# apple/ml-stable-diffusion

Measured on AMD Instinct MI355X. Metric: diffusion iter/s (UNet steps/s), SD2.1-base 512x512 fp16, higher is better.
Workload: dtype fp16; 1 GPU; BASELINE config 2: SD2.1-base (865.9 M-parameter UNet), random-init, denoising iteration at 512x512 (64x64 latents), CFG batch 2 per prompt, DDIM, device-resident loop; unet=sd21-base, latent=64, attention=ORIGINAL, prompts_per_gpu=1, global_batch=2, hip_graph=True, parallelism=dp1 (independent prompts per rank, no data-path collective)

## Files before the change

ml-stable-diffusion_amd/csrc/capi.cpp:

```cpp
#include <cmath>
#include <cstdlib>
#include <cstring>

#include "unet.h"

namespace sd {
extern thread_local std::string g_last_error;
int selftest_mfma();

namespace {

template <typename F>
int guarded(F&& f) {
  try {
    f();
    g_last_error.clear();
    return kOk;
  } catch (const Error& e) {
    g_last_error = e.what();
    return e.code;
  } catch (const std::bad_alloc&) {
    g_last_error = "out of host memory";
    return kInternal;
  } catch (const std::exception& e) {
    g_last_error = e.what();
    return kInternal;
  }
}

void require_device() {
  int n = 0;
  hipError_t e = hipGetDeviceCount(&n);
  if (e != hipSuccess || n <= 0)
    fail(kHipError, "no HIP device visible (%s): libsdmi355 has no CPU fallback", hipGetErrorString(e));
}

struct Scratch {
  std::vector<void*> ptrs;
  hipStream_t stream = nullptr;
  hipEvent_t e0 = nullptr, e1 = nullptr;
  Scratch() {
    require_device();
    SD_HIP(hipStreamCreateWithFlags(&stream, hipStreamNonBlocking));
    SD_HIP(hipEventCreate(&e0));
    SD_HIP(hipEventCreate(&e1));
  }
  ~Scratch() {
    if (stream) (void)hipStreamSynchronize(stream);
    for (void* p : ptrs) (void)hipFree(p);
    if (e0) (void)hipEventDestroy(e0);
    if (e1) (void)hipEventDestroy(e1);
    if (stream) (void)hipStreamDestroy(stream);
  }
  template <typename T>
  T* dev(size_t n, const T* host = nullptr) {
    void* p = nullptr;
    SD_HIP(hipMalloc(&p, std::max<size_t>(n, 1) * sizeof(T)));
    ptrs.push_back(p);
    if (host)
      SD_HIP(hipMemcpy(p, host, n * sizeof(T), hipMemcpyHostToDevice));
    else
      SD_HIP(hipMemset(p, 0, std::max<size_t>(n, 1) * sizeof(T)));
    return reinterpret_cast<T*>(p);
  }
  template <typename F>
  void timed(int iters, float* ms, F&& launch) {
    if (iters < 1) iters = 1;
    static const bool poison = tune_env_set("SD_POISON_LDS");
    if (poison) {
      launch();
      launch_lds_poison(stream);
      launch();
      SD_HIP(hipStreamSynchronize(stream));
      if (ms) *ms = 0.f;
      return;
    }
    launch();
    SD_HIP(hipStreamSynchronize(stream));
    static const bool cold = tune_env_set("SD_BENCH_COLD");
    if (cold) {
      const size_t flush_bytes = (size_t)512 << 20;
      void* flush = dev<char>(flush_bytes);
// ... 936 lines not shown
      auto gemm_res = [&](const half_t* in, int cin, const half_t* w, const float* bias, const half_t* res, half_t* dst) {
        ConvDesc cd;
        cd.x0 = in; cd.C0 = cin; cd.w = w; cd.bias = bias; cd.res = res; cd.out = dst;
        cd.B = B; cd.Hi = 1; cd.Wi = S; cd.Ho = 1; cd.Wo = S; cd.N = C;
        SD_REQUIRE(conv_fast_path_ok(cd), kInvalidArgument, "ffn_out_proj: off the MFMA path");
        return cd;
      };
      ConvDesc c1 = gemm_res(dg, K1, dw1, db1, dr1, dh3);
      ConvDesc c2 = gemm_res(dh3, C, dw2, db2, dr2, o);
      c2.gn_partial = partial;
      c2.gn_groups = groups;
      ConvWorkspace ws;
      ws.partial_bytes = std::max(conv_workspace_bytes(c1), conv_workspace_bytes(c2));
      if (ws.partial_bytes) ws.partial = reinterpret_cast<float*>(sc.dev<char>(ws.partial_bytes));
      sc.timed(iters, ms, [&] {
        launch_conv(c1, ws, sc.stream);
        n_entries = launch_conv(c2, ws, sc.stream);
      });
    }
    std::vector<half_t> ot((size_t)M * C);
    SD_HIP(hipMemcpy(ot.data(), o, ot.size() * 2, hipMemcpyDeviceToHost));
    half_t* oh = reinterpret_cast<half_t*>(out);
    for (int b = 0; b < B; ++b)
      for (int c = 0; c < C; ++c)
        for (int s = 0; s < S; ++s) oh[((size_t)b * C + c) * S + s] = ot[((size_t)b * S + s) * C + c];
    if (gn_sums) {
      std::vector<float> hp(pf);
      SD_HIP(hipMemcpy(hp.data(), partial, pf * sizeof(float), hipMemcpyDeviceToHost));
      for (int b = 0; b < B; ++b)
        for (int gi = 0; gi < groups; ++gi) {
          double s1 = 0.0, s2 = 0.0;
          for (int e = 0; e < n_entries; ++e) {
            s1 += hp[(((size_t)b * groups + gi) * kGnMaxSlabs + e) * 2];
            s2 += hp[(((size_t)b * groups + gi) * kGnMaxSlabs + e) * 2 + 1];
          }
          gn_sums[((size_t)b * groups + gi) * 2] = n_entries ? (float)s1 : NAN;
          gn_sums[((size_t)b * groups + gi) * 2 + 1] = n_entries ? (float)s2 : NAN;
        }
    }
  });
}

int sd_op_geglu(const void* x, const void* w, const float* bias, void* out, int M, int C, int N2, int iters, float* ms) {
  return guarded([&] {
    SD_REQUIRE(x && w && out && N2 % 2 == 0, kInvalidArgument, "bad GEGLU arguments");
    Scratch sc;
    const half_t* wh = reinterpret_cast<const half_t*>(w);
    const int half_n = N2 / 2;
    SD_REQUIRE(half_n % 32 == 0, kUnsupported, "GEGLU needs (N/2) %% 32 == 0");
    std::vector<half_t> wt((size_t)N2 * C);
    std::vector<float> bt(N2, 0.f);
    for (int o = 0; o < N2; ++o) {
      const bool gate = o >= half_n;
      const int j = gate ? o - half_n : o;
      const int dst = (j / 32) * 64 + (gate ? 32 : 0) + (j % 32);
      std::memcpy(&wt[(size_t)dst * C], &wh[(size_t)o * C], (size_t)C * 2);
      if (bias) bt[dst] = bias[o];
    }
    ConvDesc d;
    d.x0 = sc.dev<half_t>((size_t)M * C, reinterpret_cast<const half_t*>(x));
    d.C0 = C;
    d.w = sc.dev<half_t>(wt.size(), wt.data());
    d.bias = bias ? sc.dev<float>(N2, bt.data()) : nullptr;
    half_t* dout = sc.dev<half_t>((size_t)M * half_n);
    d.out = dout;
    d.B = 1; d.Hi = 1; d.Wi = M; d.Ho = 1; d.Wo = M;
    d.N = N2;
    d.out_mode = kOutGeglu;
    const bool fast = conv_fast_path_ok(d);
    ConvWorkspace ws;
    sc.timed(iters, ms, [&] {
      if (fast)
        launch_conv(d, ws, sc.stream);
      else
        launch_conv_generic(d, 0, sc.stream);
    });
    SD_HIP(hipMemcpy(out, dout, (size_t)M * half_n * 2, hipMemcpyDeviceToHost));
  });
}

int sd_op_geglu_ln(const void* x, const float* ln_weight, const float* ln_bias, const void* w, const float* bias, void* out, int M, int C,
                   int N2, float eps, int kernel, int iters, float* ms) {
  return guarded([&] {
    const int abl = kernel / 10;
    kernel %= 10;
    SD_REQUIRE(x && w && out && N2 % 64 == 0 && (ln_weight == nullptr) == (ln_bias == nullptr) && kernel >= 0 && kernel <= 9 &&
                   (abl == 0 || kernel == 2), kInvalidArgument, "bad GEGLU arguments");
    Scratch sc;
    const half_t* wh = reinterpret_cast<const half_t*>(w);
    const int half_n = N2 / 2;
    std::vector<half_t> wt((size_t)N2 * C);
    std::vector<float> bt(N2, 0.f), cst(N2, 0.f);
    for (int o = 0; o < N2; ++o) {
      const bool gate = o >= half_n;
      const int j = gate ? o - half_n : o;
      const int dst = (j / 32) * 64 + (gate ? 32 : 0) + (j % 32);
      double cs = 0.0, bb = bias ? (double)bias[o] : 0.0;
      for (int c = 0; c < C; ++c) {
        const float wv = (float)wh[(size_t)o * C + c];
        const half_t h = ln_weight ? (half_t)(wv * ln_weight[c]) : wh[(size_t)o * C + c];
        wt[(size_t)dst * C + c] = h;
        cs += (double)(float)h;
        if (ln_bias) bb += (double)wv * (double)ln_bias[c];
      }
      bt[dst] = (float)bb;
      cst[dst] = (float)cs;
    }
    ConvDesc d;
    d.x0 = sc.dev<half_t>((size_t)M * C, reinterpret_cast<const half_t*>(x));
    d.C0 = C;
    d.w = sc.dev<half_t>(wt.size(), wt.data());
    d.bias = sc.dev<float>(N2, bt.data());
    if (ln_weight) d.ln_colsum = sc.dev<float>(N2, cst.data());
    d.ln_eps = eps;
    half_t* dout = sc.dev<half_t>((size_t)M * half_n);
    d.out = dout;
    d.B = 1; d.Hi = 1; d.Wi = M; d.Ho = 1; d.Wo = M;
    d.N = N2;
    d.out_mode = kOutGeglu;
    SD_REQUIRE(conv_fast_path_ok(d), kUnsupported, "GEGLU shape off the MFMA path (C=%d N2=%d)", C, N2);
    if (kernel != 1 && kernel < 3 && wsgemm_shape_ok(d)) {
      half_t* wtd = sc.dev<half_t>(wsgemm_tiled_halves(N2));
      launch_wsgemm_retile(d.w, wtd, N2, true, sc.stream);
      d.w_ws = wtd;
    }
    if (kernel == 2) d.tile = 10;
    if (kernel >= 3) {
      SD_REQUIRE(bvgemm_shape_ok(d), kInvalidArgument, "GEGLU shape not eligible for plan tile 11 (bvgemm.hip)");
      half_t* wtd = sc.dev<half_t>(bvgemm_tiled_halves(N2, C));
      launch_bvgemm_retile(d.w, wtd, N2, C, true, sc.stream);
      d.w_bv = wtd;
      d.w_ws = nullptr;
      d.tile = 11;
      d.staging = kernel - 3;
    }
    d.debug = abl;
    if (abl == 5) d.prof = sc.dev<long long>(64);
    ConvWorkspace ws;
    sc.timed(iters, ms, [&] { launch_conv(d, ws, sc.stream); });
    if (d.prof) {
      long long t[64];
      SD_HIP(hipMemcpy(t, d.prof, sizeof(t), hipMemcpyDeviceToHost));
      for (int i = 0; i < 6; ++i)
        fprintf(stderr, "[sd prof] wsgemm iteration %d: barrier wait %lld, DMA issue + store %lld, statistics %lld, MFMA || epilogue %lld cycles\n",
                i + 1, t[i * 8 + 1] - t[i * 8], t[i * 8 + 2] - t[i * 8 + 1], t[i * 8 + 3] - t[i * 8 + 2], t[i * 8 + 4] - t[i * 8 + 3]);
    }
    SD_HIP(hipMemcpy(out, dout, (size_t)M * half_n * 2, hipMemcpyDeviceToHost));
  });
}

int sd_op_qkv_ln(const void* x, const float* ln_weight, const float* ln_bias, const void* w, void* out_qk, void* out_vt, int B, int HW, int C,
                 float eps, float q_scale, int vt_perm, int kernel, int iters, float* ms) {
  return guarded([&] {
    SD_REQUIRE(x && ln_weight && ln_bias && w && out_qk && out_vt && B >= 1 && HW >= 1 && C % 64 == 0 && kernel >= 0 && kernel <= 9,
               kInvalidArgument, "bad q|k|v arguments");
    Scratch sc;
    const half_t* wh = reinterpret_cast<const half_t*>(w);
    const int N = 3 * C, M = B * HW;
    std::vector<half_t> wt((size_t)N * C);
    std::vector<float> bt(N, 0.f), cst(N, 0.f);
    for (int o = 0; o < N; ++o) {
      double cs = 0.0, bb = 0.0;
      for (int c = 0; c < C; ++c) {
        const float wv = (float)wh[(size_t)o * C + c];
        const half_t h = (half_t)(wv * ln_weight[c]);
        wt[(size_t)o * C + c] = h;
        cs += (double)(float)h;
        bb += (double)wv * (double)ln_bias[c];
      }
      bt[o] = (float)bb;
      cst[o] = (float)cs;
    }
    ConvDesc d;
    d.x0 = sc.dev<half_t>((size_t)M * C, reinterpret_cast<const half_t*>(x));
    d.C0 = C;
    d.w = sc.dev<half_t>(wt.size(), wt.data());
    d.bias = sc.dev<float>(N, bt.data());
    d.ln_colsum = sc.dev<float>(N, cst.data());
    d.ln_eps = eps;
    half_t* dqk = sc.dev<half_t>((size_t)M * 2 * C);
    half_t* dvt = sc.dev<half_t>((size_t)B * C * HW);
    d.out = dqk;
    d.out_t = dvt;
    d.n_trans = 2 * C;
    d.ldT = HW;
    d.vt_perm = vt_perm ? 1 : 0;
    d.q_scale = q_scale;
    d.q_cols = C;
    d.B = B; d.Hi = 1; d.Wi = HW; d.Ho = 1; d.Wo = HW;
    d.N = N;
    SD_REQUIRE(conv_fast_path_ok(d), kUnsupported, "q|k|v shape off the MFMA path (C=%d)", C);
    if (kernel == 2 || (kernel == 0 && wsgemm_wanted(d))) {
      SD_REQUIRE(wsgemm_shape_ok(d), kInvalidArgument, "q|k|v shape not eligible for plan tile 10 (wsgemm.hip)");
      half_t* wtd = sc.dev<half_t>(wsgemm_tiled_halves(N));
      launch_wsgemm_retile(d.w, wtd, N, false, sc.stream);
      d.w_ws = wtd;
      if (kernel == 2) d.tile = 10;
    } else if (kernel >= 3 || (kernel == 0 && bvgemm_wanted(d))) {
      SD_REQUIRE(bvgemm_shape_ok(d), kInvalidArgument, "q|k|v shape not eligible for plan tile 11 (bvgemm.hip)");
      half_t* wtd = sc.dev<half_t>(bvgemm_tiled_halves(N, C));
      launch_bvgemm_retile(d.w, wtd, N, C, false, sc.stream);
      d.w_bv = wtd;
      if (kernel >= 3) {
        d.tile = 11;
        d.staging = kernel - 3;
      }
    }
    ConvWorkspace ws;
    sc.timed(iters, ms, [&] { launch_conv(d, ws, sc.stream); });
    SD_HIP(hipMemcpy(out_qk, dqk, (size_t)M * 2 * C * 2, hipMemcpyDeviceToHost));
    SD_HIP(hipMemcpy(out_vt, dvt, (size_t)B * C * HW * 2, hipMemcpyDeviceToHost));
  });
}

int sd_op_gn_proj_qkv(const void* x_in, const void* conv_w, const float* gn_weight, const float* gn_bias, const void* proj_w,
                      const float* proj_bias, const float* ln_weight, const float* ln_bias, const void* wqkv, void* out_h, void* out_qk,
                      void* out_vt, int B, int H, int W, int C, int groups, float gn_eps, float ln_eps, float q_scale, int vt_perm, int fused,
                      int* entries, int iters, float* ms) {
  return guarded([&] {
    SD_REQUIRE(x_in && conv_w && gn_weight && gn_bias && proj_w && proj_bias && ln_weight && ln_bias && wqkv && out_h && out_qk && out_vt,
               kInvalidArgument, "NULL argument");
    const int HW = H * W, M = B * HW, N = 3 * C;
    SD_REQUIRE(gn_proj_qkv_ok(C, C / 64, HW, M, HW, groups), kInvalidArgument, "gn_proj_qkv: C=%d HW=%d groups=%d", C, HW, groups);
// ... 276 lines not shown
```

ml-stable-diffusion_amd/csrc/igemm.hip:

```cpp
#include <cstdio>
#include <cstdlib>
#include <cstring>
#include <string>
#include <type_traits>

#include "kernels.h"

namespace sd {

namespace {

constexpr int BK = 64;
constexpr int LDS_ROW = BK + 8;

struct IgemmArgs {
  const half_t* x0;
  const half_t* x1;
  const half_t* w;
  const float* bias;
  const float* temb;
  const half_t* res;
  half_t* out;
  float* partial;
  int C0, C1, Ctot;
// ... 2407 lines not shown
    int ppb = std::max(1, a.B * a.HoWo / 512);
    const int slabs = cdiv(a.HoWo, ppb);
    const size_t lds = (size_t)ppb * (a.N / 4) * 2 * sizeof(float);
    if (slabs <= kGnMaxSlabs && lds <= 64 * 1024) {
      a.gn_partial = d.gn_partial;
      a.gn_G = d.gn_groups;
      a.gn_cpg = a.N / d.gn_groups;
      a.gn_T = slabs;
      hipLaunchKernelGGL(splitk_reduce_stats_kernel, dim3(slabs, a.B), dim3(256), lds, s, a, ppb);
      return slabs;
    }
  }
  const size_t total4 = (size_t)a.M * a.N / 4;
  const int blocks = (int)std::min<size_t>((total4 + 255) / 256, 2048);
  hipLaunchKernelGGL(splitk_reduce_kernel, dim3(blocks), dim3(256), 0, s, a);
  return 0;
}
}

namespace {
void choose_tile_order(IgemmArgs& a, int tile) {
  int bm, bn;
  tile_dims(tile, bm, bn);
  const bool halo_tile = tile == 7;
  const double nbn = (double)cdiv(a.N, bn);
  const double nbm = halo_tile ? (double)a.B * a.tiles_x * a.tiles_y : (double)cdiv(a.M, bm);
  const double a_bytes = 2.0 * a.B * a.Hi * a.Wi * a.Ctot, w_bytes = 2.0 * a.N * a.K;
  const double l2 = 3.5e6;
  const double m_fast_cost = w_bytes + a_bytes * (a_bytes <= l2 ? std::min(8.0, nbn) : nbn);
  const double n_fast_cost = a_bytes + w_bytes * (w_bytes <= l2 ? std::min(8.0, nbm) : nbm);
  static const int forced = tune_env_int("SD_TILE_ORDER", -1);
  if (forced == 2) a.n_fast = nbn > 1 && a_bytes * (nbn - 1) > 7.0 * w_bytes;
  else a.n_fast = forced >= 0 ? (forced != 0) : (nbn > 1 && n_fast_cost < m_fast_cost);
}
}

bool conv_gn_loader_ok(const ConvDesc& d) {
  const int c1 = d.x1 ? d.C1 : 0;
  const int ctot = d.C0 + c1;
  return d.ksize == 3 && d.stride == 1 && d.up == 1 && halo_ks_ok(d) && !d.ln_colsum && !d.out_t && d.out_mode == kOutHalf && !d.debug &&
         d.gnf_groups >= 1 && d.gnf_groups <= 32 && ctot % d.gnf_groups == 0 && ctot <= 2048 && d.Hi == d.Ho && d.Wi == d.Wo &&
         halo_gnl_lds_bytes(3, ctot) <= halo_gnl_lds_cap;
}

int launch_conv(const ConvDesc& d, const ConvWorkspace& ws, hipStream_t s) {
  SD_REQUIRE(conv_fast_path_ok(d), kInvalidArgument, "launch_conv: shape not MFMA-tileable (C0=%d C1=%d N=%d k=%d)",
             d.C0, d.C1, d.N, d.ksize);
  SD_REQUIRE(!d.ln_colsum || (d.ksize == 1 && !d.x1 && d.bias && d.out_mode != kOutHalfT), kInvalidArgument,
             "LayerNorm fold needs a 1x1 single-source GEMM with a (folded) bias");
  SD_REQUIRE(!d.out_t || (d.out_mode == kOutHalf && d.n_trans % 64 == 0 && d.n_trans < d.N && (d.Ho * d.Wo) % 8 == 0 &&
                          d.ldT % 8 == 0 && !d.res && !d.temb),
             kInvalidArgument, "fused q|k|v: n_trans %d N %d HoWo %d ldT %d", d.n_trans, d.N, d.Ho * d.Wo, d.ldT);
  SD_REQUIRE(!d.vt_perm || (d.out_t && (d.Ho * d.Wo) % 16 == 0), kInvalidArgument, "permuted V^T needs the fused q|k|v epilogue and HoWo %% 16 == 0");
  SD_REQUIRE(d.q_cols == 0 || (d.out_t && d.q_cols % 4 == 0 && d.q_cols <= d.n_trans), kInvalidArgument, "pre-scaled queries need the fused q|k|v epilogue (q_cols %d)", d.q_cols);
  {
    static const bool wsg_on = tune_env_int("SD_WSGEMM", 1) != 0;
    const bool forced = d.tile == 10;
    if (d.w_ws && wsgemm_shape_ok(d) && (forced || (wsg_on && wsgemm_wanted(d) && d.tile == 0 && d.splitk == 0 && d.staging == 0 && g_tune.tile == 0))) {
      launch_wsgemm(d, s);
      return 0;
    }
    SD_REQUIRE(!forced, kInvalidArgument, "plan tile 10 (wsgemm.hip) needs the pre-tiled weights and an eligible GEGLU shape");
  }
  {
    static const bool bv_on = tune_env_int("SD_BVGEMM", 1) != 0;
    if (bv_on && d.w_bv && d.tile == 0 && d.splitk == 0 && d.staging == 0 && g_tune.tile == 0 && bvgemm_wanted(d)) {
      launch_bvgemm(d, 0, s);
      return 0;
    }
  }
  if (d.tile == 11) {
    SD_REQUIRE(d.w_bv && bvgemm_shape_ok(d), kInvalidArgument, "plan tile 11 (bvgemm.hip) needs the pre-tiled weights and an eligible 1x1 shape");
    launch_bvgemm(d, d.staging, s);
    return 0;
  }
  {
    static const bool sm_on = tune_env_int("SD_SMGEMM", 1) != 0;
    const bool forced = d.tile == 12;
    if (forced || (sm_on && d.tile == 0 && d.splitk == 0 && d.staging == 0 && g_tune.tile == 0 && smgemm_wanted(d))) {
      launch_smgemm(d, forced ? d.staging : 0, s);
      return 0;
    }
  }
  IgemmArgs a = make_args(d);
  Plan p = choose_plan(d, a);
  bool halo = p.tile == 7;
  const bool twins = d.n_twins > 0;
  SD_REQUIRE(!twins || (d.out_mode == kOutHalf && !d.ln_colsum && !d.out_t && !d.debug && reduce_twin_ok(a.HoWo, a.N, d.n_twins, d.twin)),
             kInvalidArgument, "GroupNorm twins need a plain fp16 output and whole (sample, group) slices (HoWo=%d N=%d)", a.HoWo, a.N);
  if (d.gnf_partial && d.ksize == 3) {
    SD_REQUIRE(conv_gn_loader_ok(d) && d.gnf_silu == 1 && d.gnf_gamma && d.gnf_beta && d.gnf_entries >= 1 && d.gnf_entries <= 128 && !twins, kInvalidArgument,
               "GroupNorm in the conv loader: Ctot=%d groups=%d entries=%d up=%d", a.Ctot, d.gnf_groups, d.gnf_entries, d.up);
    p.tile = 7;
    if (p.staging != 2 && p.staging != 3) p.staging = 3;
    p.splitk = 1;
  } else if (d.gnf_partial) {
    SD_REQUIRE(d.ksize == 1 && d.stride == 1 && !d.x1 && d.out_mode == kOutHalf && !d.ln_colsum && !d.out_t && !twins && gemm_pipe_ok(a) &&
                   d.gnf_gamma && d.gnf_beta && d.gnf_groups >= 1 && d.gnf_groups <= 32 && a.K % d.gnf_groups == 0 && a.K <= 2048 &&
                   d.gnf_entries >= 1 && d.gnf_entries <= 128 && a.HoWo % 64 == 0,
               kInvalidArgument, "GroupNorm fold: K=%d groups=%d entries=%d HoWo=%d", a.K, d.gnf_groups, d.gnf_entries, a.HoWo);
    p.tile = 3;
    if (p.staging != 6 && p.staging != 7 && p.staging != 8) p.staging = 6;
    p.splitk = 1;
  }
  halo = p.tile == 7;
  if (p.tile == 9) {
    const int nw = p.staging == 4 ? 4 : 8;
    const int S = wstream_splits(d, nw);
    const size_t need = (size_t)S * a.M * a.N * sizeof(float);
    SD_REQUIRE(ws.partial && ws.partial_bytes >= need, kInternal, "wstream workspace too small (%zu < %zu)", ws.partial_bytes, need);
    static const bool log_ws = tune_env_set("SD_LOG_CONVS");
    if (log_ws)
      fprintf(stderr, "[sd conv] k%d up%d C0=%d C1=%d M=%d N=%d K=%d tile=9 nw=%d slabs=%d twins=%d\n", a.ksize, a.up, a.C0, a.C1, a.M, a.N,
              a.K, nw, S, d.n_twins);
    launch_wstream(d, ws.partial, nw, s);
    a.partial = ws.partial;
    a.splitk = S;
    a.slab = 1;
    int entries = 0;
    if (twins) launch_reduce_twin(a.partial, S, a.M, a.N, a.HoWo, a.bias, a.temb, a.temb_stride, a.res, a.out, d.n_twins, d.twin, s);
    else entries = launch_slab_combine(d, a, s);
    SD_HIP(hipGetLastError());
    return entries;
  }
  if (halo) {
    const int nch = a.Ctot / BK;
    a.nk_per_split = cdiv(nch, p.splitk);
    a.splitk = cdiv(nch, a.nk_per_split);
  } else {
    a.splitk = p.splitk;
    a.nk_per_split = cdiv(a.nk_total, p.splitk);
    a.splitk = cdiv(a.nk_total, a.nk_per_split);
  }
  a.slab = (a.splitk > 1 || twins) ? 1 : 0;
  if (a.slab) {
    size_t need = (size_t)a.splitk * a.M * a.N * sizeof(float);
    SD_REQUIRE(ws.partial && ws.partial_bytes >= need, kInternal, "split-K workspace too small (%zu < %zu)",
               ws.partial_bytes, need);
    a.partial = ws.partial;
  }
  const bool trans = d.out_mode == kOutHalfT;
  const int st = p.staging;
  choose_tile_order(a, p.tile);
  static const bool log_plans = tune_env_set("SD_LOG_CONVS");
  if (log_plans)
    fprintf(stderr, "[sd conv] k%d s%d up%d C0=%d C1=%d M=%d N=%d K=%d mode=%d tile=%d splitk=%d\n", a.ksize, a.stride, a.up,
            a.C0, a.C1, a.M, a.N, a.K, d.out_mode, p.tile, a.splitk);
  int gn_entries = 0;
  if (halo) {
    gn_entries = setup_gn_stats(d, a, 0);
    launch_halo_ks(a, a.splitk, st, s);
  } else if (d.debug && d.debug < 64) {
    const bool ok = p.tile == 1 ? launch_debug_mode<128, 128>(a, d.debug, s) : launch_debug_mode<64, 64>(a, d.debug, s);
    SD_REQUIRE(ok && !trans, kInvalidArgument, "no ablation kernel for debug mode %d", d.debug);
    return 0;
  } else {
    if (!trans) {
      int bm, bn;
      tile_dims(p.tile >= 1 && p.tile <= 3 ? p.tile : 4, bm, bn);
      gn_entries = setup_gn_stats(d, a, bm);
    }
    switch (p.tile) {
      case 1: launch_tile<128, 128, 2, 2>(a, trans, st, s); break;
      case 2: launch_tile<128, 64, 2, 2>(a, trans, st, s); break;
      case 3: launch_tile<64, 64, 2, 2>(a, trans, st, s); break;
      default: launch_tile<64, 128, 2, 2>(a, trans, st, s); break;
// ... 117 lines not shown
```

ml-stable-diffusion_amd/csrc/kernels.h:

```cpp
#pragma once
#include "sd_common.h"

namespace sd {

enum OutMode : int {
  kOutHalf = 0,
  kOutHalfT = 1,
  kOutGeglu = 2,
};

struct GnTwin {
  half_t* y = nullptr;
  int ld = 0, c_off = 0;
  int cpg = 0;
  const float* gamma = nullptr;
  const float* beta = nullptr;
  float eps = 1e-5f;
  int silu = 0;
};

struct ConvDesc {
  const half_t* x0 = nullptr;
  const half_t* x1 = nullptr;
  int C0 = 0, C1 = 0;
  const half_t* w = nullptr;
  const float* bias = nullptr;
  const float* temb = nullptr;
  int temb_stride = 0;
  const half_t* res = nullptr;
  half_t* out = nullptr;
  int B = 1, Hi = 1, Wi = 1;
  int Ho = 1, Wo = 1;
  int ksize = 1, stride = 1, up = 1;
  int pad = -1;
  int N = 0;
  int out_mode = kOutHalf;
  int ldT = 0;
  int tile = 0;
  int splitk = 0;
  long long* prof = nullptr;
  int debug = 0;
  int staging = 0;
  const float* ln_colsum = nullptr;
  float ln_eps = 1e-5f;
  half_t* out_t = nullptr;
  int n_trans = 0;
  int vt_perm = 0;
  float q_scale = 1.f;
  int q_cols = 0;
  float* gn_partial = nullptr;
  int gn_groups = 0;
  const float* gnf_partial = nullptr;
  const float* gnf_gamma = nullptr;
  const float* gnf_beta = nullptr;
  float gnf_eps = 1e-6f;
  int gnf_groups = 0, gnf_entries = 0;
  int gnf_silu = 0;
  const half_t* w_tiled = nullptr;
  const half_t* w_ws = nullptr;
  const half_t* w_bv = nullptr;
  GnTwin twin[2];
  int n_twins = 0;
};

constexpr int kGnMaxSlabs = 256;

struct ConvWorkspace {
  float* partial = nullptr;
  size_t partial_bytes = 0;
};

size_t conv_workspace_bytes(const ConvDesc& d);
int launch_conv(const ConvDesc& d, const ConvWorkspace& ws, hipStream_t s);
bool conv_fast_path_ok(const ConvDesc& d);
bool conv_gn_loader_ok(const ConvDesc& d);
void conv_tune_set_candidate(int tile, int staging, int splitk);
int conv_plan_table_set(const char* text);

bool conv_plan_is_wstream(const ConvDesc& d);
bool wstream_shape_ok(const ConvDesc& d);
int wstream_splits(const ConvDesc& d, int nw);
size_t wstream_tiled_halves(int N, int Ctot, int ksize);
void launch_wstream_retile(const half_t* w, half_t* wt, int N, int Ctot, int ksize, hipStream_t s);
int launch_wstream(const ConvDesc& d, float* partial, int nw, hipStream_t s);
bool reduce_twin_ok(int HW, int N, int n_twins, const GnTwin* tw);
void launch_reduce_twin(const float* partial, int S, int M, int N, int HW, const float* bias, const float* temb, int temb_stride,
                        const half_t* res, half_t* out, int n_twins, const GnTwin* tw, hipStream_t s);

bool wsgemm_shape_ok(const ConvDesc& d);
bool wsgemm_wanted(const ConvDesc& d);
size_t wsgemm_tiled_halves(int N);
void launch_wsgemm_retile(const half_t* w, half_t* wt, int N, bool geglu, hipStream_t s);
void launch_wsgemm(const ConvDesc& d, hipStream_t s);

bool bvgemm_shape_ok(const ConvDesc& d);
size_t bvgemm_tiled_halves(int N, int K);
void launch_bvgemm_retile(const half_t* w, half_t* wt, int N, int K, bool geglu, hipStream_t s);
void launch_bvgemm(const ConvDesc& d, int variant, hipStream_t s);
bool bvgemm_wanted(const ConvDesc& d);

bool smgemm_shape_ok(const ConvDesc& d, int variant);
bool smgemm_wanted(const ConvDesc& d);
void launch_smgemm(const ConvDesc& d, int variant, hipStream_t s);

void run_calibration(int device, float* out);

int launch_conv_generic(const ConvDesc& d, int act_silu_out, hipStream_t s);

void launch_conv_small_n(const ConvDesc& d, float* out_nchw_f32, hipStream_t s);

enum AttnImpl : int { kAttnOriginal = 0, kAttnSplitEinsum = 1, kAttnSplitEinsumV2 = 2 };

struct AttnDesc {
  const half_t* q = nullptr;
  const half_t* k = nullptr;
  const half_t* vt = nullptr;
  half_t* out = nullptr;
  int B = 1, heads = 1, d = 64, Sq = 0, Sk = 0;
  int ldq = 0, ldk = 0, ldv = 0, ldo = 0;
  int impl = kAttnOriginal;
  int variant = 0;
  int vt_perm = 0;
  int q_prescaled = 0;
  float* sk_part = nullptr;
  size_t sk_part_bytes = 0;
  unsigned* sk_cnt = nullptr;
  int sk_cnt_n = 0;
  int sk_force = 0;
  int sk_upw = 0;
};
inline float attention_q_prescale(int d) { return 1.4426950408889634f / sqrtf((float)d); }
void launch_attention(const AttnDesc& d, hipStream_t s);
bool attention_supported(int d);
bool attention8_ok(const AttnDesc& d);
bool attention8_shape_ok(int d, int Sq, int Sk);
void launch_attention8(const AttnDesc& d, hipStream_t s);
bool attention8_sk_scratch(const AttnDesc& d, size_t* part_bytes, int* n_counters);

struct XAttnDesc {
  const half_t* x = nullptr;
  const half_t* wq = nullptr;
  const float* bias = nullptr;
  const float* colsum = nullptr;
  const half_t* k = nullptr;
  const half_t* vt = nullptr;
  half_t* out = nullptr;
  int M = 0, C = 0, S = 0, L = 0, ldv = 0, heads = 0;
  float ln_eps = 1e-5f;
  int impl = kAttnOriginal;
  int nst = 0;
};
bool xattn_fused_ok(int C, int heads, int S, int L);
void launch_xattn_fused(const XAttnDesc& d, hipStream_t s);

struct XAttnOutDesc {
  const half_t* x = nullptr;
  const half_t* wq_t = nullptr;
  const float* q_bias = nullptr;
  const float* q_colsum = nullptr;
  const half_t* k = nullptr;
  const half_t* vt = nullptr;
  const half_t* wo_t = nullptr;
  const float* o_bias = nullptr;
  half_t* out = nullptr;
  int M = 0, C = 0, S = 0, L = 0, ldv = 0, heads = 0;
  float ln_eps = 1e-5f;
  int impl = kAttnOriginal;
  const half_t* h0 = nullptr;
  const half_t* wo1_t = nullptr;
  const float* o1_bias = nullptr;
};
struct GnProjQkvDesc {
  const half_t* x = nullptr;
  const float* gn_partial = nullptr;
  const float* gn_gamma = nullptr;
  const float* gn_beta = nullptr;
  int gn_entries = 0, gn_groups = 32;
  float gn_eps = 1e-6f;
  const half_t* wp_t = nullptr;
  const float* p_bias = nullptr;
  half_t* h = nullptr;
  const half_t* wqkv_t = nullptr;
  const float* qkv_bias = nullptr;
  const float* qkv_colsum = nullptr;
  float ln_eps = 1e-5f;
  half_t* qk = nullptr;
  half_t* vt = nullptr;
// ... 97 lines not shown
```

ml-stable-diffusion_amd/csrc/smgemm.hip:

```cpp
#include <algorithm>

#include "kernels.h"

namespace sd {

namespace {

constexpr int SM_BK = 64;
constexpr int SM_BN = 80;
constexpr int SM_NW = SM_BN / 16;
constexpr int SM_LDS = 160 * 1024;

struct SmArgs {
  const half_t* x;
  const half_t* w;
  const float* bias;
  const half_t* res;
  half_t* out;
  int K, N, nk, res_ld;
  int has_bias, has_res;
  unsigned per_xcd;
  unsigned fast_div;
  unsigned fast_magic;
  int n_fast;
};

template <int BM>
struct SmCfg {
  static constexpr int ROWS = SM_BN + BM;
  static constexpr int PIECES = ROWS / 8;
  static constexpr int PPW = (PIECES + SM_NW - 1) / SM_NW;
  static constexpr int STAGE = SM_NW * PPW * 1024;
  static constexpr int NST = SM_LDS / STAGE;
  static constexpr int TM = BM / 16;
  static constexpr int EPI = 1 + TM / 2;
  static_assert(BM % 32 == 0 && ROWS % 8 == 0, "tile");
  static_assert(NST >= 3 && NST * STAGE <= SM_LDS, "ring");
  static_assert(PPW * (NST - 2) + EPI <= 63, "vmcnt range");
};

template <int N>
__device__ __forceinline__ void sm_wait_barrier() {
  asm volatile("s_waitcnt vmcnt(%0)\n\ts_barrier" ::"n"(N) : "memory");
}

template <int PPW, int E, int A>
__device__ __forceinline__ void sm_wait(int ahead) {
  if constexpr (A > 0) {
    if (ahead == A) {
      sm_wait_barrier<PPW * A + E>();
      return;
    }
    sm_wait<PPW, E, A - 1>(ahead);
  } else {
    sm_wait_barrier<E>();
  }
}

template <int BM>
__global__ __launch_bounds__(64 * SM_NW, 1) void smgemm_kernel(SmArgs a) {
  using C = SmCfg<BM>;
  constexpr int NST = C::NST, PPW = C::PPW, TM = C::TM;
  extern __shared__ __attribute__((aligned(16))) char smem[];
  const int lane = threadIdx.x & 63;
  const int wave = __builtin_amdgcn_readfirstlane((int)threadIdx.x >> 6);

  const unsigned t = (blockIdx.x & 7u) * a.per_xcd + (blockIdx.x >> 3);
  const unsigned slow = __umulhi(t, a.fast_magic);
  const unsigned fast = t - slow * a.fast_div;
  const int m_blk = (int)(a.n_fast ? slow : fast) * BM;
  const int n_blk = (int)(a.n_fast ? fast : slow) * SM_BN;

  const half_t* src[PPW];
#pragma unroll
  for (int j = 0; j < PPW; ++j) {
    const int r = (wave + SM_NW * j) * 8 + (lane >> 3);
    const int chunk = (lane & 7) ^ ((r >> 1) & 7);
    int rx = r - SM_BN;
    if (rx >= BM) rx -= BM;
    src[j] = (r < SM_BN ? a.w + (size_t)(n_blk + r) * a.K : a.x + (size_t)(m_blk + rx) * a.K) + chunk * 8;
  }
  auto issue = [&](int idx) {
    char* st = smem + (idx % NST) * C::STAGE + wave * 1024;
#pragma unroll
    for (int j = 0; j < PPW; ++j) {
      __builtin_amdgcn_global_load_lds((const __attribute__((address_space(1))) void*)src[j],
                                       (__attribute__((address_space(3))) void*)(st + j * SM_NW * 1024), 16, 0, 0);
      src[j] += SM_BK;
    }
  };

#pragma unroll
  for (int p = 0; p < NST - 1; ++p)
    if (p < a.nk) issue(p);
  const int g = lane >> 4, r16 = lane & 15;
  __builtin_amdgcn_sched_barrier(0);
  const floatx4 bias4 = *reinterpret_cast<const floatx4*>(a.bias + n_blk + 16 * wave + 4 * g);
  half8 resv[TM / 2];
#pragma unroll
  for (int p = 0; p < TM / 2; ++p)
    resv[p] = *reinterpret_cast<const half8*>(a.res + (size_t)(m_blk + 32 * p + 16 * (g & 1) + r16) * a.res_ld + n_blk + 16 * wave +
                                              8 * (g >> 1));
  __builtin_amdgcn_sched_barrier(0);

  int foff[2];
#pragma unroll
  for (int kk = 0; kk < 2; ++kk) foff[kk] = r16 * 128 + (((4 * kk + g) ^ ((r16 >> 1) & 7)) * 16);

  floatx4 acc[TM];
#pragma unroll
  for (int i = 0; i < TM; ++i) acc[i] = floatx4{0.f, 0.f, 0.f, 0.f};

  for (int rel = 0; rel < a.nk; ++rel) {
    const int ahead = min(NST - 2, a.nk - 1 - rel);
    if (rel <= NST - 2) sm_wait<PPW, C::EPI, NST - 2>(ahead);
    else sm_wait<PPW, 0, NST - 2>(ahead);
    const char* st = smem + (rel % NST) * C::STAGE;
    half8 wf[2], xf[2][TM];
#pragma unroll
    for (int kk = 0; kk < 2; ++kk) {
      wf[kk] = *reinterpret_cast<const half8*>(st + 16 * wave * 128 + foff[kk]);
#pragma unroll
      for (int i = 0; i < TM; ++i) xf[kk][i] = *reinterpret_cast<const half8*>(st + (SM_BN + 16 * i) * 128 + foff[kk]);
    }
    __builtin_amdgcn_sched_barrier(0);
    if (rel + NST - 1 < a.nk) issue(rel + NST - 1);
#pragma unroll
    for (int kk = 0; kk < 2; ++kk)
#pragma unroll
      for (int i = 0; i < TM; ++i)
        acc[i] = __builtin_amdgcn_mfma_f32_16x16x32_f16(wf[kk], xf[kk][i], acc[i], 0, 0, 0);
  }

  const floatx4 bv = a.has_bias ? bias4 : floatx4{0.f, 0.f, 0.f, 0.f};
  const int n = n_blk + 16 * wave + 8 * (g >> 1);
#pragma unroll
  for (int p = 0; p < TM / 2; ++p) {
    unsigned lo[2], hi[2];
#pragma unroll
    for (int b = 0; b < 2; ++b) {
// ... 93 lines not shown
```

Baseline: 236.5 it/s.

## Add multi-stage LDS-ring GEGLU GEMM kernel with fused LayerNorm fold

Adds a new GEGLU projection kernel (plan tile 13) that streams weight and activation tiles into a deep LDS ring with direct global-to-LDS loads and counted vmcnt waits. It computes the value and gate MFMAs together, accumulates LayerNorm row statistics from the staged activations, and applies the bias, LayerNorm fold and erf-GELU gating in the epilogue. Dispatch selects it by default for shapes whose tile count falls in a set window, with an env switch to disable it. The aim is to keep loads overlapped with MFMA work and to reduce launch and tail costs of the GEGLU GEMMs, at the cost of a large single-wave-per-CU LDS footprint and a polynomial erf approximation.

```diff
diff --git a/ml-stable-diffusion_amd/csrc/capi.cpp b/ml-stable-diffusion_amd/csrc/capi.cpp
--- a/ml-stable-diffusion_amd/csrc/capi.cpp
+++ b/ml-stable-diffusion_amd/csrc/capi.cpp
@@ -1,3 +1,5 @@
+#include <algorithm>
+#include <climits>
 #include <cmath>
 #include <cstdlib>
 #include <cstring>
@@ -1100,6 +1102,10 @@
 int sd_op_geglu_ln(const void* x, const float* ln_weight, const float* ln_bias, const void* w, const float* bias, void* out, int M, int C,
                    int N2, float eps, int kernel, int iters, float* ms) {
   return guarded([&] {
+    const bool smgeglu = kernel >= 100 && kernel <= 112 && kernel % 10 <= 2;
+    const int sg_variant = smgeglu ? kernel % 10 : 0;
+    const bool sg_clock = smgeglu && kernel >= 110;
+    if (smgeglu) kernel = 0;
     const int abl = kernel / 10;
     kernel %= 10;
     SD_REQUIRE(x && w && out && N2 % 64 == 0 && (ln_weight == nullptr) == (ln_bias == nullptr) && kernel >= 0 && kernel <= 9 &&
@@ -1136,14 +1142,24 @@
     d.B = 1; d.Hi = 1; d.Wi = M; d.Ho = 1; d.Wo = M;
     d.N = N2;
     d.out_mode = kOutGeglu;
+    SD_REQUIRE(!smgeglu || smgeglu_shape_ok(d, sg_variant), kInvalidArgument,
+               "GEGLU shape not eligible for plan tile 13 (smgeglu.hip): M=%d C=%d N2=%d", M, C, N2);
     SD_REQUIRE(conv_fast_path_ok(d), kUnsupported, "GEGLU shape off the MFMA path (C=%d N2=%d)", C, N2);
-    if (kernel != 1 && kernel < 3 && wsgemm_shape_ok(d)) {
+    if (kernel != 1 && kernel < 3 && !smgeglu && wsgemm_shape_ok(d)) {
       half_t* wtd = sc.dev<half_t>(wsgemm_tiled_halves(N2));
       launch_wsgemm_retile(d.w, wtd, N2, true, sc.stream);
       d.w_ws = wtd;
     }
     if (kernel == 2) d.tile = 10;
-    if (kernel >= 3) {
+    size_t sg_prof = 0;
+    if (smgeglu) {
+      d.tile = 13;
+      d.staging = sg_variant;
+      if (sg_clock) {
+        sg_prof = smgeglu_prof_entries(d, d.staging);
+        d.prof = sc.dev<long long>(sg_prof);
+      }
+    } else if (kernel >= 3) {
       SD_REQUIRE(bvgemm_shape_ok(d), kInvalidArgument, "GEGLU shape not eligible for plan tile 11 (bvgemm.hip)");
       half_t* wtd = sc.dev<half_t>(bvgemm_tiled_halves(N2, C));
       launch_bvgemm_retile(d.w, wtd, N2, C, true, sc.stream);
@@ -1156,7 +1172,26 @@
     if (abl == 5) d.prof = sc.dev<long long>(64);
     ConvWorkspace ws;
     sc.timed(iters, ms, [&] { launch_conv(d, ws, sc.stream); });
-    if (d.prof) {
+    if (sg_prof) {
+      std::vector<long long> t(sg_prof);
+      SD_HIP(hipMemcpy(t.data(), d.prof, sg_prof * sizeof(long long), hipMemcpyDeviceToHost));
+      static const char* const phase[5] = {"first ring stages + epilogue operands issued", "first stage landed (counted wait + barrier)",
+                                           "K loop done", "row statistics exchanged", "last store issued"};
+      const size_t waves = sg_prof / 8;
+      fprintf(stderr, "[sd prof] smgeglu M=%d K=%d N=%d kernel=%d: %zu waves, shader-clock cycles since the wave's kernel entry (min / mean / max)\n",
+              M, C, N2, 110 + sg_variant, waves);
+      for (int k = 1; k <= 5; ++k) {
+        long long lo = LLONG_MAX, hi = 0;
+        double sum = 0.0;
+        for (size_t wv = 0; wv < waves; ++wv) {
+          const long long dt = t[wv * 8 + k] - t[wv * 8];
+          lo = std::min(lo, dt);
+          hi = std::max(hi, dt);
+          sum += (double)dt;
+        }
+        fprintf(stderr, "[sd prof]   %-46s %8lld %10.0f %8lld\n", phase[k - 1], lo, sum / (double)waves, hi);
+      }
+    } else if (d.prof) {
       long long t[64];
       SD_HIP(hipMemcpy(t, d.prof, sizeof(t), hipMemcpyDeviceToHost));
       for (int i = 0; i < 6; ++i)
diff --git a/ml-stable-diffusion_amd/csrc/igemm.hip b/ml-stable-diffusion_amd/csrc/igemm.hip
--- a/ml-stable-diffusion_amd/csrc/igemm.hip
+++ b/ml-stable-diffusion_amd/csrc/igemm.hip
@@ -2513,6 +2513,14 @@
       return 0;
     }
   }
+  {
+    static const bool sg_on = tune_env_int("SD_SMGEGLU", 1) != 0;
+    const bool forced = d.tile == 13;
+    if (forced || (sg_on && d.tile == 0 && d.splitk == 0 && d.staging == 0 && g_tune.tile == 0 && smgeglu_wanted(d))) {
+      launch_smgeglu(d, forced ? d.staging : 0, s);
+      return 0;
+    }
+  }
   IgemmArgs a = make_args(d);
   Plan p = choose_plan(d, a);
   bool halo = p.tile == 7;
diff --git a/ml-stable-diffusion_amd/csrc/kernels.h b/ml-stable-diffusion_amd/csrc/kernels.h
--- a/ml-stable-diffusion_amd/csrc/kernels.h
+++ b/ml-stable-diffusion_amd/csrc/kernels.h
@@ -103,6 +103,11 @@
 bool smgemm_wanted(const ConvDesc& d);
 void launch_smgemm(const ConvDesc& d, int variant, hipStream_t s);
 
+bool smgeglu_shape_ok(const ConvDesc& d, int variant);
+bool smgeglu_wanted(const ConvDesc& d);
+void launch_smgeglu(const ConvDesc& d, int variant, hipStream_t s);
+size_t smgeglu_prof_entries(const ConvDesc& d, int variant);
+
 void run_calibration(int device, float* out);
 
 int launch_conv_generic(const ConvDesc& d, int act_silu_out, hipStream_t s);
diff --git a/ml-stable-diffusion_amd/csrc/sm_ring.h b/ml-stable-diffusion_amd/csrc/sm_ring.h
--- /dev/null
+++ b/ml-stable-diffusion_amd/csrc/sm_ring.h
@@ -0,0 +1,23 @@
+#pragma once
+
+namespace sd {
+
+template <int N>
+__device__ __forceinline__ void sm_wait_barrier() {
+  asm volatile("s_waitcnt vmcnt(%0)\n\ts_barrier" ::"n"(N) : "memory");
+}
+
+template <int PPW, int E, int A>
+__device__ __forceinline__ void sm_wait(int ahead) {
+  if constexpr (A > 0) {
+    if (ahead == A) {
+      sm_wait_barrier<PPW * A + E>();
+      return;
+    }
+    sm_wait<PPW, E, A - 1>(ahead);
+  } else {
+    sm_wait_barrier<E>();
+  }
+}
+
+}
diff --git a/ml-stable-diffusion_amd/csrc/smgeglu.hip b/ml-stable-diffusion_amd/csrc/smgeglu.hip
--- /dev/null
+++ b/ml-stable-diffusion_amd/csrc/smgeglu.hip
@@ -0,0 +1,372 @@
+#include <algorithm>
+
+#include "kernels.h"
+#include "sm_ring.h"
+
+namespace sd {
+
+namespace {
+
+constexpr int SG_BK = 64;
+constexpr int SG_UNITS = 5;
+constexpr int SG_WROWS = 32 * SG_UNITS;
+constexpr int SG_BN = 16 * SG_UNITS;
+constexpr int SG_NW = 2 * SG_UNITS;
+constexpr int SG_LDS = 160 * 1024;
+constexpr int SG_STAMPS = 8;
+
+struct SgArgs {
+  const half_t* x;
+  const half_t* w;
+  const float* bias;
+  const float* colsum;
+  half_t* out;
+  long long* prof;
+  int K, nk, ldo;
+  int has_bias, lnf;
+  float ln_eps;
+  unsigned per_xcd;
+  unsigned fast_div;
+  unsigned fast_magic;
+  int n_fast;
+};
+
+template <int BM>
+struct SgCfg {
+  static constexpr int ROWS = SG_WROWS + BM;
+  static constexpr int PIECES = ROWS / 8;
+  static constexpr int PPW = (PIECES + SG_NW - 1) / SG_NW;
+  static constexpr int FULL = PIECES - SG_NW * (PPW - 1);
+  static constexpr int STAGE = PIECES * 1024;
+  static constexpr int NST = (SG_LDS - BM * 8) / STAGE;
+  static constexpr int TM = BM / 32;
+  static constexpr int SB = TM / 4;
+  static constexpr int EPI = 4;
+  static constexpr size_t LDS = (size_t)NST * STAGE + BM * 8;
+  static_assert(BM % 128 == 0 && ROWS % 8 == 0 && PPW >= 2 && FULL >= 1 && FULL <= SG_NW, "tile");
+  static_assert(NST >= 3 && LDS <= SG_LDS, "ring");
+  static_assert(PPW * (NST - 2) + EPI <= 63, "vmcnt range");
+};
+
+__device__ __forceinline__ float sg_gelu_erf(float x) {
+  const float z = x * 0.70710678118654752f;
+  const float az = fabsf(z);
+  const float t = __builtin_amdgcn_rcpf(fmaf(0.3275911f, az, 1.0f));
+  float p = 1.061405429f;
+  p = fmaf(p, t, -1.453152027f);
+  p = fmaf(p, t, 1.421413741f);
+  p = fmaf(p, t, -0.284496736f);
+  p = fmaf(p, t, 0.254829592f);
+  const float e = __builtin_amdgcn_exp2f(-az * az * 1.4426950408889634f);
+  const float erf_abs = fmaf(-p * t, e, 1.0f);
+  return 0.5f * x * (1.0f + copysignf(erf_abs, z));
+}
+
+__device__ __forceinline__ int sg_unit_row(int U) { return 64 * (U >> 1) + 16 * (U & 1); }
+
+template <int BM, bool PROF>
+__global__ __launch_bounds__(64 * SG_NW, 1) void smgeglu_kernel(SgArgs a) {
+  using C = SgCfg<BM>;
+  constexpr int NST = C::NST, PPW = C::PPW, TM = C::TM, SB = C::SB;
+  extern __shared__ __attribute__((aligned(16))) char smem[];
+  long long stamp[6] = {};
+  if constexpr (PROF) stamp[0] = clock64();
+  const int lane = threadIdx.x & 63;
+  const int wave = __builtin_amdgcn_readfirstlane((int)threadIdx.x >> 6);
+  const int u = wave % SG_UNITS, h = wave / SG_UNITS;
+
+  const unsigned t = (blockIdx.x & 7u) * a.per_xcd + (blockIdx.x >> 3);
+  const unsigned slow = __umulhi(t, a.fast_magic);
+  const unsigned fast = t - slow * a.fast_div;
+  const int m_blk = (int)(a.n_fast ? slow : fast) * BM;
+  const int u_blk = (int)(a.n_fast ? fast : slow) * SG_UNITS;
+
+  const bool full = wave < C::FULL;
+  const half_t* src[PPW];
+  int pdst[PPW];
+#pragma unroll
+  for (int j = 0; j < PPW; ++j) {
+    int p = wave + SG_NW * j;
+    if (p >= C::PIECES) p -= C::PIECES;
+    pdst[j] = p * 1024;
+    const int r = p * 8 + (lane >> 3);
+    const int chunk = (lane & 7) ^ ((r >> 1) & 7);
+    const int wrow = sg_unit_row(u_blk + (r >> 5)) + 2 * (r & 16) + (r & 15);
+    src[j] = (r < SG_WROWS ? a.w + (size_t)wrow * a.K : a.x + (size_t)(m_blk + r - SG_WROWS) * a.K) + chunk * 8;
+  }
+  auto issue = [&](int slot) {
+    char* st = smem + slot * C::STAGE;
+#pragma unroll
+    for (int j = 0; j < PPW; ++j) {
+      if (j == PPW - 1 && !full) break;
+      __builtin_amdgcn_global_load_lds((const __attribute__((address_space(1))) void*)src[j],
+                                       (__attribute__((address_space(3))) void*)(st + pdst[j]), 16, 0, 0);
+      src[j] += SG_BK;
+    }
+  };
+
+#pragma unroll
+  for (int p = 0; p < NST - 1; ++p)
+    if (p < a.nk) issue(p);
+  const int g = lane >> 4, r16 = lane & 15;
+  const int vrow = sg_unit_row(u_blk + u) + 4 * g;
+  __builtin_amdgcn_sched_barrier(0);
+  const floatx4 bias_v = *reinterpret_cast<const floatx4*>(a.bias + vrow);
+  const floatx4 bias_g = *reinterpret_cast<const floatx4*>(a.bias + vrow + 32);
+  const floatx4 cs_v = *reinterpret_cast<const floatx4*>(a.colsum + vrow);
+  const floatx4 cs_g = *reinterpret_cast<const floatx4*>(a.colsum + vrow + 32);
+  __builtin_amdgcn_sched_barrier(0);
+  if constexpr (PROF) stamp[1] = clock64();
+
+  int foff[2];
+#pragma unroll
+  for (int kk = 0; kk < 2; ++kk) foff[kk] = r16 * 128 + (((4 * kk + g) ^ ((r16 >> 1) & 7)) * 16);
+  const int w_off = 32 * u * 128;
+  const int x_off = (SG_WROWS + h * (BM / 2)) * 128;
+
+  floatx4 accv[TM], accg[TM];
+#pragma unroll
+  for (int i = 0; i < TM; ++i) accv[i] = accg[i] = floatx4{0.f, 0.f, 0.f, 0.f};
+  float ln_s1[SB], ln_s2[SB];
+#pragma unroll
+  for (int s = 0; s < SB; ++s) ln_s1[s] = ln_s2[s] = 0.f;
+  const half2v one2 = {(half_t)1.f, (half_t)1.f};
+
+  constexpr int NG = TM / 4, NQ = 2 * NG;
+  half8 wv[2], wg[2], wvn[2], wgn[2], xq[2][4];
+  auto read_w = [&](const char* st, half8 (&v)[2], half8 (&gt)[2]) {
+#pragma unroll
+    for (int kk = 0; kk < 2; ++kk) {
+      v[kk] = *reinterpret_cast<const half8*>(st + w_off + foff[kk]);
+      gt[kk] = *reinterpret_cast<const half8*>(st + w_off + 16 * 128 + foff[kk]);
+    }
+  };
+  auto read_q = [&](const char* st, int q) {
+#pragma unroll
+    for (int i = 0; i < 4; ++i)
+      xq[q & 1][i] = *reinterpret_cast<const half8*>(st + x_off + 16 * (4 * (q % NG) + i) * 128 + foff[q / NG]);
+  };
+  auto wait_stage = [&](int s) {
+    const int ahead = min(NST - 2, a.nk - 1 - s);
+    if (full) {
+      if (s <= NST - 2) sm_wait<PPW, C::EPI, NST - 2>(ahead);
+      else sm_wait<PPW, 0, NST - 2>(ahead);
+    } else {
+      if (s <= NST - 2) sm_wait<PPW - 1, C::EPI, NST - 2>(ahead);
+      else sm_wait<PPW - 1, 0, NST - 2>(ahead);
+    }
+  };
+
+  wait_stage(0);
+  if constexpr (PROF) stamp[2] = clock64();
+  if (NST - 1 < a.nk) issue(NST - 1);
+  read_w(smem, wv, wg);
+  read_q(smem, 0);
+  __builtin_amdgcn_sched_barrier(0);
+  int slot = 0;
+  for (int rel = 0; rel < a.nk; ++rel) {
+    const char* st = smem + slot * C::STAGE;
+    const int nslot = slot + 1 == NST ? 0 : slot + 1;
+#pragma unroll
+    for (int q = 0; q < NQ; ++q) {
+      const int kk = q / NG;
+      const bool next_stage = q + 1 == NQ && rel + 1 < a.nk;
+      if (next_stage) {
+        asm volatile("s_waitcnt lgkmcnt(0)" ::: "memory");
+        wait_stage(rel + 1);
+        if (rel + NST < a.nk) issue(slot);
+      }
+      __builtin_amdgcn_sched_barrier(0);
+      accv[4 * (q % NG)] = __builtin_amdgcn_mfma_f32_16x16x32_f16(wv[kk], xq[q & 1][0], accv[4 * (q % NG)], 0, 0, 0);
+      __builtin_amdgcn_sched_barrier(0);
+      if (q + 1 < NQ) {
+        read_q(st, q + 1);
+      } else if (next_stage) {
+        read_w(smem + nslot * C::STAGE, wvn, wgn);
+        read_q(smem + nslot * C::STAGE, 0);
+      }
+      __builtin_amdgcn_sched_barrier(0);
+#pragma unroll
+      for (int i = 0; i < 4; ++i) {
+        const int blk = 4 * (q % NG) + i;
+        if (i > 0) accv[blk] = __builtin_amdgcn_mfma_f32_16x16x32_f16(wv[kk], xq[q & 1][i], accv[blk], 0, 0, 0);
+        accg[blk] = __builtin_amdgcn_mfma_f32_16x16x32_f16(wg[kk], xq[q & 1][i], accg[blk], 0, 0, 0);
+      }
+      if (a.lnf) {
+#pragma unroll
+        for (int i = 0; i < 4; ++i) {
+          const int blk = 4 * (q % NG) + i;
+          if (blk / SB == u) {
+#pragma unroll
+            for (int e = 0; e < 4; ++e) {
+              const half2v p2 = {xq[q & 1][i][2 * e], xq[q & 1][i][2 * e + 1]};
+              ln_s2[blk % SB] = __builtin_amdgcn_fdot2(p2, p2, ln_s2[blk % SB], false);
+              ln_s1[blk % SB] = __builtin_amdgcn_fdot2(p2, one2, ln_s1[blk % SB], false);
+            }
+          }
+        }
+      }
+      __builtin_amdgcn_sched_barrier(0);
+    }
+#pragma unroll
+    for (int kk = 0; kk < 2; ++kk) wv[kk] = wvn[kk], wg[kk] = wgn[kk];
+    slot = nslot;
+  }
+  if constexpr (PROF) stamp[3] = clock64();
+
+  float ln_a[TM], ln_b[TM];
+  if (a.lnf) {
+    float2* stat = reinterpret_cast<float2*>(smem + NST * C::STAGE);
+    const float inv_k = 1.0f / (float)a.K;
+#pragma unroll
+    for (int s = 0; s < SB; ++s) {
+      float s1 = ln_s1[s], s2 = ln_s2[s];
+      s1 += __shfl_xor(s1, 16);
+      s2 += __shfl_xor(s2, 16);
+      s1 += __shfl_xor(s1, 32);
+      s2 += __shfl_xor(s2, 32);
+      const float mean = s1 * inv_k;
+      const float var = fmaxf(s2 * inv_k - mean * mean, 0.f);
+      const float la = rsqrtf(var + a.ln_eps);
+      if (u < 4 && g == 0) stat[h * (BM / 2) + 16 * (u * SB + s) + r16] = make_float2(la, -la * mean);
+    }
+    __syncthreads();
+#pragma unroll
+    for (int i = 0; i < TM; ++i) {
+      const float2 ab = stat[h * (BM / 2) + 16 * i + r16];
+      ln_a[i] = ab.x;
+      ln_b[i] = ab.y;
+    }
+  } else {
+#pragma unroll
+    for (int i = 0; i < TM; ++i) ln_a[i] = 1.f, ln_b[i] = 0.f;
+  }
+  if constexpr (PROF) stamp[4] = clock64();
+
+  const floatx4 zero4 = {0.f, 0.f, 0.f, 0.f};
+  const floatx4 bv = a.has_bias ? bias_v : zero4, bg = a.has_bias ? bias_g : zero4;
+  const int n = (u_blk + u) * 16 + 8 * (g >> 1);
+#pragma unroll
+  for (int p = 0; p < TM / 2; ++p) {
+    unsigned lo[2], hi[2];
+#pragma unroll
+    for (int b = 0; b < 2; ++b) {
+      const int i = 2 * p + b;
+      float o[4];
+#pragma unroll
+      for (int e = 0; e < 4; ++e) {
+        float v, gt;
+        if (a.lnf) {
+          v = fmaf(accv[i][e], ln_a[i], fmaf(ln_b[i], cs_v[e], bv[e]));
+          gt = fmaf(accg[i][e], ln_a[i], fmaf(ln_b[i], cs_g[e], bg[e]));
+        } else {
+          v = accv[i][e] + bv[e];
+          gt = accg[i][e] + bg[e];
+        }
+        o[e] = v * sg_gelu_erf(gt);
+      }
+      const half2v h01 = {(half_t)o[0], (half_t)o[1]};
+      const half2v h23 = {(half_t)o[2], (half_t)o[3]};
+      lo[b] = __builtin_bit_cast(unsigned, h01);
+      hi[b] = __builtin_bit_cast(unsigned, h23);
+    }
+    const auto s0 = __builtin_amdgcn_permlane16_swap(lo[0], lo[1], false, false);
+    const auto s1 = __builtin_amdgcn_permlane16_swap(hi[0], hi[1], false, false);
+    const unsigned d0 = s0[0], d1 = s1[0], d2 = s0[1], d3 = s1[1];
+    typedef unsigned u4 __attribute__((ext_vector_type(4)));
+    const half8 o8 = __builtin_bit_cast(half8, (u4){d0, d1, d2, d3});
+    const int m = m_blk + h * (BM / 2) + 32 * p + 16 * (g & 1) + r16;
+    out_store(reinterpret_cast<half8*>(a.out + (size_t)m * a.ldo + n), o8);
+  }
+  if constexpr (PROF) {
+    stamp[5] = clock64();
+    if (lane == 0) {
+      long long* dst = a.prof + ((size_t)blockIdx.x * SG_NW + wave) * SG_STAMPS;
+#pragma unroll
+      for (int k = 0; k < 6; ++k) dst[k] = stamp[k];
+    }
+  }
+}
+
+int sg_bm(const ConvDesc& d, int variant) {
+  if (variant == 1) return 128;
+  if (variant == 2) return 256;
+  const long M = (long)d.B * d.Ho * d.Wo;
+  return M % 128 == 0 && M / 128 * (d.N / SG_WROWS) <= 256 ? 128 : 256;
+}
+
+template <int BM, bool PROF>
+void sg_launch(const SgArgs& a, unsigned nwg, hipStream_t s) {
+  auto k = smgeglu_kernel<BM, PROF>;
+  static DynLdsOnce once;
+  once.set(k, SgCfg<BM>::LDS);
+  hipLaunchKernelGGL(k, dim3(nwg), dim3(64 * SG_NW), SgCfg<BM>::LDS, s, a);
+}
+
+}
+
+size_t smgeglu_prof_entries(const ConvDesc& d, int variant) {
+  const long M = (long)d.B * d.Ho * d.Wo;
+  return (size_t)(M / sg_bm(d, variant) * (d.N / SG_WROWS)) * SG_NW * SG_STAMPS;
+}
+
+bool smgeglu_shape_ok(const ConvDesc& d, int variant) {
+  if (!(d.ksize == 1 && d.stride == 1 && d.up == 1 && !d.x1 && d.out_mode == kOutGeglu && !d.out_t && !d.temb && !d.res &&
+        d.q_cols == 0 && !d.gnf_partial && !d.gn_partial && d.n_twins == 0 && !d.debug && (!d.ln_colsum || d.bias) && variant >= 0 &&
+        variant <= 2))
+    return false;
+  const long M = (long)d.B * d.Ho * d.Wo;
+  const int bm = sg_bm(d, variant);
+  const long mt = M / bm, nt = d.N / SG_WROWS;
+  return d.C0 % SG_BK == 0 && d.C0 >= SG_BK && d.N % SG_WROWS == 0 && d.N % 64 == 0 && M % bm == 0 && mt >= 2 && nt >= 2 &&
+         (mt * nt) % 8 == 0 && mt * nt <= 65535;
+}
+
+bool smgeglu_wanted(const ConvDesc& d) {
+  if (!smgeglu_shape_ok(d, 0)) return false;
+  const long M = (long)d.B * d.Ho * d.Wo;
+  const long tiles = M / sg_bm(d, 0) * (d.N / SG_WROWS);
+  return tiles >= 192 && tiles <= 256;
+}
+
+void launch_smgeglu(const ConvDesc& d, int variant, hipStream_t s) {
+  SD_REQUIRE(smgeglu_shape_ok(d, variant), kInvalidArgument,
+             "plan tile 13 (smgeglu.hip): not a single-source 1x1 GEGLU projection it tiles (C0=%d N=%d M=%d)", d.C0, d.N, d.B * d.Ho * d.Wo);
+  const int M = d.B * d.Ho * d.Wo, K = d.C0;
+  const int bm = sg_bm(d, variant);
+  const unsigned mt = M / bm, nt = d.N / SG_WROWS, nwg = mt * nt;
+  SgArgs a;
+  a.x = d.x0;
+  a.w = d.w;
+  a.bias = d.bias ? d.bias : reinterpret_cast<const float*>(d.w);
+  a.colsum = d.ln_colsum ? d.ln_colsum : a.bias;
+  a.out = d.out;
+  a.prof = d.prof;
+  a.K = K;
+  a.nk = K / SG_BK;
+  a.ldo = d.N / 2;
+  a.has_bias = d.bias != nullptr;
+  a.lnf = d.ln_colsum != nullptr;
+  a.ln_eps = d.ln_eps;
+  a.per_xcd = nwg / 8;
+  const double a_bytes = 2.0 * M * K, w_bytes = 2.0 * d.N * K, l2 = 3.5e6;
+  const double m_fast_cost = w_bytes + a_bytes * (a_bytes <= l2 ? std::min(8.0, (double)nt) : (double)nt);
+  const double n_fast_cost = a_bytes + w_bytes * (w_bytes <= l2 ? std::min(8.0, (double)mt) : (double)mt);
+  a.n_fast = n_fast_cost < m_fast_cost;
+  a.fast_div = a.n_fast ? nt : mt;
+  a.fast_magic = (unsigned)((1ull << 32) / a.fast_div + 1);
+  static const bool log_plans = tune_env_set("SD_LOG_CONVS");
+  if (log_plans)
+    fprintf(stderr, "[sd conv] k1 s1 up1 C0=%d C1=0 M=%d N=%d K=%d mode=%d tile=13 bm=%d n_fast=%d\n", d.C0, M, d.N, K, d.out_mode, bm,
+            a.n_fast);
+  if (bm == 128) {
+    if (d.prof) sg_launch<128, true>(a, nwg, s);
+    else sg_launch<128, false>(a, nwg, s);
+  } else {
+    if (d.prof) sg_launch<256, true>(a, nwg, s);
+    else sg_launch<256, false>(a, nwg, s);
+  }
+  SD_HIP(hipGetLastError());
+}
+
+}
diff --git a/ml-stable-diffusion_amd/csrc/smgemm.hip b/ml-stable-diffusion_amd/csrc/smgemm.hip
--- a/ml-stable-diffusion_amd/csrc/smgemm.hip
+++ b/ml-stable-diffusion_amd/csrc/smgemm.hip
@@ -1,6 +1,7 @@
 #include <algorithm>
 
 #include "kernels.h"
+#include "sm_ring.h"
 
 namespace sd {
 
@@ -38,24 +39,6 @@
   static_assert(NST >= 3 && NST * STAGE <= SM_LDS, "ring");
   static_assert(PPW * (NST - 2) + EPI <= 63, "vmcnt range");
 };
-
-template <int N>
-__device__ __forceinline__ void sm_wait_barrier() {
-  asm volatile("s_waitcnt vmcnt(%0)\n\ts_barrier" ::"n"(N) : "memory");
-}
-
-template <int PPW, int E, int A>
-__device__ __forceinline__ void sm_wait(int ahead) {
-  if constexpr (A > 0) {
-    if (ahead == A) {
-      sm_wait_barrier<PPW * A + E>();
-      return;
-    }
-    sm_wait<PPW, E, A - 1>(ahead);
-  } else {
-    sm_wait_barrier<E>();
-  }
-}
 
 template <int BM>
 __global__ __launch_bounds__(64 * SM_NW, 1) void smgemm_kernel(SmArgs a) {
```

After: 240.0 it/s, median of 6. 1.5% higher.
